# LLNL/ppo_and_friends

Measured on AMD Instinct MI355X. Metric: env_steps_per_sec, higher is better.
Workload: dtype f32; 1 GPU; C2 CartPole-v1 MLP (4->128x3->2 actor, ->1 critic), envs_per_proc=4096, ts_per_rollout=128, fixed-length synthetic trajectories, batch_size=256, epochs_per_iter=10; parallelism=dp1, hip_graphs=True

## Files before the change

### ppo_and_friends_amd/csrc/ppo_update.hip

```cpp
#include "ppo_update_rowpair.hpp"
#include <hip/hip_ext.h>
#include "peer_exchange_device.hpp"
#include <cstdlib>

namespace ppoaf {


template <int HTA, int HTC, bool SPLIT>
__global__ __launch_bounds__(kThreadsU) void ppo_update_fwd_bwd_kernel(UpdateDev u) {
    const int b = blockIdx.x;
    int which = (b >> 2) & 1;
    int g = ((b >> 3) << 2) | (b & 3);
    if (u.confine) {
        const int x = b & 7;
        if ((x >> 2) != u.confine - 1) return;
        which = (x & 3) >> 1;
        g = ((b >> 3) << 1) | (x & 1);
    }
    if (g >= u.n_wg) return;
    if (which == 0) ppo_update_fwd_bwd_body<HTA, SPLIT>(u, 0, g);
    else ppo_update_fwd_bwd_body<HTC, SPLIT>(u, 1, g);
}

template <int HTA, int HTC>
__global__ __launch_bounds__(kThreadsU) void ppo_update_fwd_bwd_pair_kernel(UpdateDev u, PairDev pd) {
    const int b = blockIdx.x, x = b & 7, j = b >> 3;
    int which, g, hf = 0;
    if (u.confine) {
        if ((x >> 2) != u.confine - 1) return;
        which = (x & 3) >> 1;
        if (which == 0 ? HTA == 16 : HTC == 16) { hf = j & 1; g = ((j >> 1) << 1) | (x & 1); }
        else g = (j << 1) | (x & 1);
    } else {
        which = x >> 2;
        if (which == 0 ? HTA == 16 : HTC == 16) { hf = j & 1; g = ((j >> 1) << 2) | (x & 3); }
        else g = (j << 2) | (x & 3);
    }
    if (g >= u.n_wg) return;
    if (which == 0) {
        if constexpr (HTA == 16) ppo_update_fwd_bwd_pair_body<16>(u, 0, g, hf, pd);
        else ppo_update_fwd_bwd_body<HTA, true>(u, 0, g);
    } else {
        if constexpr (HTC == 16) ppo_update_fwd_bwd_pair_body<16>(u, 1, g, hf, pd);
        else ppo_update_fwd_bwd_body<HTC, true>(u, 1, g);
    }
}

constexpr int kRedThreads = 256;

__device__ __forceinline__ void ppo_update_bookkeeping(const UpdateDev& u);

__global__ __launch_bounds__(kRedThreads) void ppo_update_reduce_kernel(UpdateDev u, int compute_norms) {
    __shared__ double red[17];
    if (blockIdx.x == gridDim.x - 1) { ppo_update_bookkeeping(u); return; }
    const long n4 = u.bucket_total >> 2;
    const long idx = (long)blockIdx.x * kRedThreads + threadIdx.x;
    const float4* sl = reinterpret_cast<const float4*>(u.slabs);
    float4 acc = make_float4(0.f, 0.f, 0.f, 0.f);
    if (idx < n4) {
        for (int g0 = 0; g0 < u.n_wg; g0 += 8) {
            float4 v[8];
#pragma unroll
            for (int k = 0; k < 8; ++k)
                v[k] = (g0 + k < u.n_wg) ? sl[(long)(g0 + k) * n4 + idx] : make_float4(0.f, 0.f, 0.f, 0.f);
#pragma unroll
            for (int k = 0; k < 8; ++k) { acc.x += v[k].x; acc.y += v[k].y; acc.z += v[k].z; acc.w += v[k].w; }
        }
// ... 465 lines not shown
```

### ppo_and_friends_amd/csrc/ppo_update_rowtile.hpp

```cpp
#pragma once
#include "ppo_update_dev.hpp"

namespace ppoaf {

extern __shared__ __attribute__((aligned(16))) unsigned char ppo_update_smem[];

#ifdef PPOAF_STAMPS
#ifndef PPOAF_STAMP_BLOCK
#define PPOAF_STAMP_BLOCK 0
#endif
static __device__ unsigned long long g_ppo_update_stamps[2][16];
#define PPOAF_STAMP(k)                                                                   \
    do {                                                                                 \
        if (blockIdx.x == PPOAF_STAMP_BLOCK && threadIdx.x == 0) {                       \
            unsigned long long t_;                                                       \
            asm volatile("s_memtime %0\n\ts_waitcnt lgkmcnt(0)" : "=s"(t_)::"memory");    \
            g_ppo_update_stamps[0][k] = t_;                                              \
        }                                                                                \
    } while (0)
#else
#define PPOAF_STAMP(k) do {} while (0)
#endif



template <int HT, bool NT>
__device__ __forceinline__ void load_fwd_set(const float* __restrict__ W, int n0, int lane, float4 (&fr)[HT]) {
    if constexpr (NT) load_fwd_frags<HT, true>(W, n0, lane, fr);
    else load_fwd_lines_buf<HT>(W, n0, lane, fr);
}
template <int HT, bool NT>
__device__ __forceinline__ f32x4 mfma_fwd_set(const float* __restrict__ A, int HS, int lane, const float4 (&fr)[HT], float init,
                                              float* __restrict__ scratch) {
    if constexpr (NT) return mfma_rows_x_frags<HT>(A, HS, lane, fr, init);
    else return mfma_rows_x_lines<HT>(A, HS, lane, fr, init, scratch);
}

template <int HT, bool SPLIT = false>
__device__ __forceinline__ void ppo_update_fwd_bwd_body(const UpdateDev& u, const int which, const int g) {
    constexpr bool NT = false;
    constexpr long mb_extra = 0;
    constexpr int H = 16 * HT, HS = H + 4;
    int tid_ = threadIdx.x;
    if (NT) {
        asm volatile("" : "+v"(tid_));
        __builtin_assume(tid_ >= 0 && tid_ < kThreadsU);
    }
    const int tid = tid_, lane = tid & 63, wave = NT ? __builtin_amdgcn_readfirstlane(tid >> 6) : (tid >> 6);
    const auto& nd = u.net[which];
    const int in_dim = nd.in_dim, depth = nd.depth, out_dim = nd.out_dim, act = nd.act;
    const int NT0 = (in_dim + 15) >> 4;
    const int INP = 16 * NT0 + 4;
    const float* P = u.params + nd.offset;
    const long B = u.B;
    const long mb = u.cursor[0] + u.mb_offset + mb_extra;
    const long base = mb * u.batch_stride;
    const long szW0 = ((long)H * in_dim + 3) & ~3L;
    auto offW = [&](int l) -> long { return l == 0 ? 0 : szW0 + H + (long)(l - 1) * (H * H + H); };
    auto offB = [&](int l) -> long {
        return l == 0 ? szW0 : offW(l) + (l < depth ? (long)H * H : (((long)out_dim * H + 3) & ~3L));
    };
    float* slab = SPLIT ? u.sp.outpart[which] + (long)g * (nd.size - offW(depth)) - offW(depth)
// ... 7 lines not shown
    };
    const long sp_plane = SPLIT ? (long)u.sp.Bp * H : 0;

    PPOAF_STAMP(0);
    int zl = 0;
    if (NT) asm volatile("" : "+s"(zl));
    float* smem = reinterpret_cast<float*>(ppo_update_smem + zl);
    int* sRow = reinterpret_cast<int*>(smem);
    float* sMisc = smem + 16;
    float* sRowF = smem + 32;
    float* sActF = smem + 80;
    float* sBias = smem + 208;
    float* sWout = sBias + (depth + 1) * H;
    float* sX = sWout + 8 * H;
    float* sH = sX + kRows * INP;
    float* sD0 = sH + (long)depth * kRows * HS;
    float* sD1 = sD0 + kRows * HS;
    float* sOut = sD1 + kRows * HS;
    float* sDOut = sOut + kRows * kMaxOut;
    float* sScr = sDOut + kRows * kMaxOut + wave * 2 * kLineSlot;

    if (!NT && g == 0 && which == 0 && tid == 0) { u.norm_scratch[0] = 0.0; u.norm_scratch[1] = 0.0; }

    const bool has_tile = wave < HT;
    const bool deep = depth == 3 && HT <= kNW;
    float4 fr[HT], fr2[HT];
    const bool l0_pre = in_dim <= 16 && HT <= kNW && has_tile;
    float l0w[4] = {0.f, 0.f, 0.f, 0.f};
    float l2_touch = 0.f;
    constexpr int kCopyRegs = 4;
    float bias_reg[kCopyRegs], wout_reg[kCopyRegs];
    const int n_bias = (depth + 1) * H, n_wout = out_dim * H;
    const bool copy_fits = n_bias <= kCopyRegs * kThreadsU && n_wout <= kCopyRegs * kThreadsU;
    auto request_weights = [&]() {
        if (NT && deep && has_tile) {
            load_fwd_set<HT, NT>(P + offW(1), wave * 16, lane, fr);
            load_fwd_set<HT, NT>(P + offW(2), wave * 16, lane, fr2);
        }
        if (l0_pre) {
            const float* w = P + offW(0) + (long)(wave * 16 + (lane & 15)) * in_dim;
#pragma unroll
            for (int j = 0; j < 4; ++j) { const int k = 4 * j + (lane >> 4); if (k < in_dim) l0w[j] = ld1<NT>(w + k); }
        }
#ifndef PPOAF_L2_TOUCH_MAX_HT
#define PPOAF_L2_TOUCH_MAX_HT 8
#endif
        if (!deep && !NT && HT <= PPOAF_L2_TOUCH_MAX_HT) for (long i = (long)tid * 32; i < nd.size; i += (long)kThreadsU * 32) l2_touch += P[i];
        if (copy_fits) {
#pragma unroll
            for (int r = 0; r < kCopyRegs; ++r) {
                const int i = tid + r * kThreadsU;
                bias_reg[r] = 0.f; wout_reg[r] = 0.f;
                if (i < n_bias) { const int l = i / H, j = i - l * H; if (l < depth || j < out_dim) bias_reg[r] = ld1<NT>(P + offB(l) + j); }
                if (i < n_wout) wout_reg[r] = ld1<NT>(P + offW(depth) + i);
            }
        }
        if (!NT && deep && has_tile) {
            load_fwd_set<HT, NT>(P + offW(1), wave * 16, lane, fr);
            load_fwd_set<HT, NT>(P + offW(2), wave * 16, lane, fr2);
        }
    };
    const float* x_src = which == 0 ? u.obs : u.critic_obs;
    const bool x_pre = !NT && u.pregathered && kRows * in_dim <= 2 * kThreadsU;
    float xr[2] = {0.f, 0.f};
    if (x_pre) {
#pragma unroll
        for (int q = 0; q < 2; ++q) {
            const int idx = tid + q * kThreadsU;
            if (idx < kRows * in_dim && (long)g * kRows + idx / in_dim < B) xr[q] = x_src[(base + (long)g * kRows) * in_dim + idx];
        }
    }
    if (!NT) request_weights();

    if (tid < kRows) {
        const long s = (long)g * kRows + tid;
        int row = -1;
        long di = -1;
        if (s < B) {
            const long p = u.perm[base + s];
            if (p >= 0 && p < u.n_rows) row = u.row_map ? u.row_map[p] : (int)p;
            di = u.pregathered ? base + s : row;
        }
        float av = 0.f, lpo = 0.f, rt = 0.f;
        if (di >= 0) {
            if (which == 0) {
                av = u.adv[di]; lpo = u.old_lp[di];
                if (u.head_kind == PPOAF_HEAD_CATEGORICAL)
                    reinterpret_cast<int*>(sActF)[tid * 8] = (int)reinterpret_cast<const int64_t*>(u.raw_actions)[di];
                else if (u.head_kind == PPOAF_HEAD_MULTI_CATEGORICAL)
                    for (int j = 0; j < u.n_slices; ++j)
                        reinterpret_cast<int*>(sActF)[tid * 8 + j] =
                            (int)reinterpret_cast<const int64_t*>(u.raw_actions)[(long)di * u.n_slices + j];
                else
                    for (int d = 0; d < out_dim; ++d)
                        sActF[tid * 8 + d] = reinterpret_cast<const float*>(u.raw_actions)[(long)di * out_dim + d];
            } else {
                rt = u.rtg[di];
            }
        }
        sRow[tid] = row;
        sRowF[tid] = av; sRowF[16 + tid] = lpo; sRowF[32 + tid] = rt;
    }

    if (tid == 64) {
        if (which == 0) {
            float mean_f = 0.f, std_f = 1.f;
            if (u.normalize_adv) {
                const double* rec = u.adv_records + mb * 3;
                mean_f = (float)rec[1];
                std_f = (float)sqrt(rec[2] / (rec[0] - 1.0));
            }
            sMisc[0] = mean_f; sMisc[1] = std_f;
        } else {
            const int slot = (int)(mb & 1);
            float m = ld1<NT>(u.vn_mean + slot), v = ld1<NT>(u.vn_var + slot);
            double cnt = ld1<NT>(u.vn_count + slot);
            if (u.normalize_values) {
                double n = 0.0, bm = 0.0, M2 = 0.0;
                for (int r = 0; r < u.n_ranks; ++r) {
                    const double* rec = u.vn_records + (mb * u.n_ranks + r) * 3;
                    const double nb = rec[0];
                    if (nb <= 0.0) continue;
                    const double d = rec[1] - bm, nn = n + nb;
                    bm += d * (nb / nn);
                    M2 += rec[2] + d * d * n * nb / nn;
                    n = nn;
                }
                if (n > 0.0) {
                    const float batch_mean = (float)bm, batch_var = (float)(M2 / n);
                    const float delta = batch_mean - m;
                    const double new_count = cnt + n;
                    const float new_mean = (float)((double)m + (double)delta * (n / new_count));
                    const double m_2 = (double)v * cnt + (double)batch_var * n +
                                       (double)(delta * delta) * cnt * n / (cnt + n);
                    m = new_mean; v = (float)(m_2 / (cnt + n)); cnt = new_count;
                }
            }
            sMisc[2] = m; sMisc[3] = v;
            if (g == 0) { u.vn_mean[slot ^ 1] = m; u.vn_var[slot ^ 1] = v; u.vn_count[slot ^ 1] = cnt; }
        }
    }
    if (copy_fits) {
#pragma unroll
        for (int r = 0; r < kCopyRegs; ++r) {
            const int i = tid + r * kThreadsU;
            if (i < n_bias) sBias[i] = bias_reg[r];
            if (i < n_wout) sWout[i] = wout_reg[r];
        }
    } else {
        for (int l = 0; l <= depth; ++l) {
            const int n = (l == depth) ? out_dim : H;
            const float* bb = P + offB(l);
            for (int i = tid; i < n; i += kThreadsU) sBias[l * H + i] = ld1<NT>(bb + i);
        }
        for (int i = tid; i < out_dim * H; i += kThreadsU) sWout[i] = ld1<NT>(P + offW(depth) + i);
    }
    for (int i = tid; i < kRows * INP; i += kThreadsU) sX[i] = 0.f;
    __syncthreads();
    PPOAF_STAMP(1);

    if (x_pre) {
#pragma unroll
        for (int q = 0; q < 2; ++q) {
            const int idx = tid + q * kThreadsU;
            const int s = idx / in_dim, i = idx - s * in_dim;
            if (idx < kRows * in_dim && sRow[s] >= 0) sX[s * INP + i] = xr[q];
        }
    } else {
        const float* src = x_src;
        for (int idx = tid; idx < kRows * in_dim; idx += kThreadsU) {
            const int s = idx / in_dim, i = idx - s * in_dim;
            const int row = sRow[s];
            const long di = u.pregathered ? base + (long)g * kRows + s : row;
            if (row >= 0) sX[s * INP + i] = src[di * in_dim + i];
        }
    }
    if (!deep && depth > 1 && has_tile) load_fwd_set<HT, NT>(P + offW(1), wave * 16, lane, fr);
    __syncthreads();
    PPOAF_STAMP(2);
    if (SPLIT) {
        float* xb = u.sp.xbuf[which] + (long)g * kRows * 64;
        for (int i = tid; i < kRows * 64; i += kThreadsU) {
            const int r = i >> 6, c = i & 63;
            xb[i] = c < 16 * NT0 ? sX[r * INP + c] : 0.f;
        }
    }

    for (int nt = wave; nt < HT; nt += kNW) {
        const int o = nt * 16 + (lane & 15);
        const float bv = sBias[o];
        f32x4 acc = {bv, bv, bv, bv};
        const float* w = P + offW(0) + (long)o * in_dim;
        const float* arow = sX + (lane & 15) * INP;
        for (int k0 = 0; k0 < in_dim; k0 += 16) {
            float bq[4];
#pragma unroll
// ... 159 lines not shown
        if (l == depth - 1) PPOAF_STAMP(12);
        __syncthreads();
        if (l == depth - 1) PPOAF_STAMP(13);
        float* t = Dc; Dc = Dn; Dn = t;
    }
    PPOAF_STAMP(8);

    if (SPLIT) {
        publish_rows(Dc, u.sp.dbuf[which]);
    } else {
        for (int mt = wave; mt < HT; mt += kNW)
            wgrad_mtile(Dc, HS, sX, INP, mt * 16, NT0, in_dim, lane, slab + offW(0), in_dim);
        for (int o = tid; o < H; o += kThreadsU) {
            float acc = 0.f;
#pragma unroll
            for (int s = 0; s < kRows; ++s) acc += Dc[s * HS + o];
            slab[offB(0) + o] = acc;
        }
    }
    if (l2_touch == 1.2345e38f) u.loss_partials[0] = l2_touch;
    PPOAF_STAMP(9);
}

constexpr size_t kRowtileLineFloats = (size_t)kNW * 2 * kLineSlot;
inline size_t rowtile_lds_floats(const NetDev& n) {
    const size_t HS = n.H + 4, INP = 16 * ((n.in_dim + 15) / 16) + 4;
    return 208 + (size_t)(n.depth + 1) * n.H + 8 * (size_t)n.H + kRows * INP + (size_t)n.depth * kRows * HS + 2 * kRows * HS +
           2 * kRows * kMaxOut;
}

}
```

### ppo_and_friends_amd/csrc/ppo_update_tail.hip

```cpp
#include "ppo_update_dev.hpp"
#include "tail_sync.hpp"
#include "peer_exchange_device.hpp"
#include <hip/hip_ext.h>
#include <cstddef>

namespace ppoaf {

constexpr int kTailMaxE = 9;

struct TailBc { long long t; double bc1, bc2s; };
__device__ __forceinline__ TailBc tail_bc_load(const UpdateDev& u, const TailDev& td, const int which) {
    TailBc r;
    r.t = td.ctl->bc_t[which];
    r.bc1 = td.ctl->bc[2 * which];
    r.bc2s = td.ctl->bc[2 * which + 1];
    return r;
}

__device__ __forceinline__ void tail_sync_wave0(const UpdateDev& u, const TailDev& td, const unsigned tag, const int b, const int which,
                                                const long long t_next, const TailBc& pre, const float lr, const double q,
                                                float* s_coef) {
    if (threadIdx.x == 0) tail_publish(td, tag, b, q);
    double bc1 = pre.bc1, bc2s = pre.bc2s;
    if (pre.t != t_next) {
        bc1 = 1.0 - pow((double)u.beta1, (double)t_next);
        bc2s = sqrt(1.0 - pow((double)u.beta2, (double)t_next));
    }
    double sq0, sq1;
    tail_gather(td, tag, sq0, sq1);
    if (threadIdx.x == 0) {
        const float total_norm = (float)sqrt(which ? sq1 : sq0);
        float coef = 1.0f;
        if (u.max_norm > 0.f) coef = fminf(u.max_norm / (total_norm + 1e-6f), 1.0f);
        s_coef[0] = u.grad_scale * coef;
        s_coef[1] = (float)((double)lr / bc1);
        s_coef[2] = (float)bc2s;
    }
}

constexpr int kTailTileFloats = 528;
struct TailXchg { XchgDev x; long long seq, wait_ticks; long seg_base[2]; };

__device__ __forceinline__ __amdgpu_buffer_rsrc_t tail_slot_rsrc(const void* base) {
    return __builtin_amdgcn_make_buffer_rsrc(const_cast<void*>(base), 0, 0xFFFFFFFF, 0x00020000);
}
__device__ __forceinline__ void tail_xchg_publish_wait(const TailXchg& c, const unsigned g) {
    asm volatile("s_waitcnt vmcnt(0)" ::: "memory");
    __syncthreads();
    const XchgDev& x = c.x;
    if (threadIdx.x == 0) {
#pragma unroll
        for (int p = 0; p < kMaxPeers; ++p)
            if (p < x.n_ranks && p != x.rank)
                __hip_atomic_store(&x.peer_flags[p][g * kMaxPeers + x.rank], c.seq, __ATOMIC_RELAXED, __HIP_MEMORY_SCOPE_SYSTEM);
    }
    const int p = (int)threadIdx.x - 64;
    if (p >= 0 && p < x.n_ranks && p != x.rank) {
        long long budget = c.wait_ticks;
        if (__hip_atomic_load(&x.words[3], __ATOMIC_RELAXED, __HIP_MEMORY_SCOPE_AGENT) != 0) budget = 0;
        const long long* flag = &x.my_flags[g * kMaxPeers + p];
        const long long t0 = (long long)wall_clock64();
        while (__hip_atomic_load(flag, __ATOMIC_RELAXED, __HIP_MEMORY_SCOPE_SYSTEM) < c.seq) {
            __builtin_amdgcn_s_sleep(1);
            if ((long long)wall_clock64() - t0 > budget) {
                __hip_atomic_store(&x.words[3], c.seq, __ATOMIC_RELAXED, __HIP_MEMORY_SCOPE_AGENT);
// ... 32 lines not shown
}
__device__ __forceinline__ float tail_xchg_sum1(const TailXchg& c, const long off, const float own) {
    const long fo = (c.seq & 1) * c.x.n4 * 4 + off;
    float acc = 0.f;
#pragma unroll
    for (int p0 = 0; p0 < kMaxPeers; p0 += 8) {
        if (p0 >= c.x.n_ranks) break;
        float v[8];
#pragma unroll
        for (int k = 0; k < 8; ++k) {
            const int p = p0 + k;
            if (p >= c.x.n_ranks) v[k] = 0.f;
            else if (p == c.x.rank) v[k] = own;
            else v[k] = __uint_as_float(__hip_atomic_load(reinterpret_cast<const unsigned*>(reinterpret_cast<const float*>(c.x.peer_slots[p]) + fo),
                                                          __ATOMIC_RELAXED, __HIP_MEMORY_SCOPE_SYSTEM));
        }
#pragma unroll
        for (int k = 0; k < 8; ++k) if (p0 + k < c.x.n_ranks) acc += v[k];
    }
    return acc;
}

struct TailPmv { float p, m, v; };
__device__ __forceinline__ TailPmv tail_pmv_load(const UpdateDev& u, const long idx, const bool ok) {
    TailPmv r = {0.f, 0.f, 0.f};
    if (ok) { r.p = u.params[idx]; r.m = u.exp_avg[idx]; r.v = u.exp_avg_sq[idx]; }
    return r;
}
__device__ __forceinline__ void tail_adam1(const UpdateDev& u, const long idx, const float g, const TailPmv& s, const TailCoef& c) {
    const float gi = g * c.gs;
    const float m = u.beta1 * s.m + (1.0f - u.beta1) * gi;
    const float v = u.beta2 * s.v + (1.0f - u.beta2) * gi * gi;
    const_cast<float*>(u.params)[idx] = s.p - c.step_size * (m / (sqrtf(v) / c.bc2_sqrt + u.adam_eps));
    u.exp_avg[idx] = m;
    u.exp_avg_sq[idx] = v;
}

template <int H, bool XCHG>
__device__ __forceinline__ void tail_job(const UpdateDev& u, const TailDev& td, const unsigned tag, const int b, const int which,
                                         const int job, float* sFold , float* sTile ,
                                         double* s_red, float* s_coef, const TailXchg* xc) {
    constexpr int MAXC = 8;
    const int tid = threadIdx.x, lane = tid & 63;
    const int wave = __builtin_amdgcn_readfirstlane(tid >> 6);
    const auto& nd = u.net[which];
    const int in_dim = nd.in_dim, depth = nd.depth, out_dim = nd.out_dim;
    const int B = (int)u.B;
    const long plane = (long)u.sp.Bp * H;
    const long szW0 = ((long)H * in_dim + 3) & ~3L;
    auto offW = [&](int l) -> long { return l == 0 ? 0 : szW0 + H + (long)(l - 1) * ((long)H * H + H); };
    auto offB = [&](int l) -> long {
        return l == 0 ? szW0 : offW(l) + (l < depth ? (long)H * H : (((long)out_dim * H + 3) & ~3L));
    };
    const long nb = nd.offset;
    float* G = u.grads + nb;
    const long long t_next = (long long)u.step_counts[which] + 1;
    const float lr = u.lr[0];
    const TailBc pre = tail_bc_load(u, td, which);
    constexpr int t = H / 16, t2 = (t + 1) / 2;
    const int n_it0 = (in_dim + 15) / 16, p0 = (n_it0 + 1) / 2;
    const int n_hidden = (depth - 1) * t * t2, n_l0 = t * p0;
    const float sc = u.grad_scale;
    double q = 0.0;
    TAIL_STAMP(td, 0);
    if (job < n_hidden + n_l0) {
        int l, ot, itile, n_it;
        if (job < n_hidden) { l = 1 + job / (t * t2); const int jj = job % (t * t2); ot = jj / t2; itile = 2 * (jj % t2); n_it = t; }
        else { l = 0; const int jj = job - n_hidden; ot = jj / p0; itile = 2 * (jj % p0); n_it = n_it0; }
        const bool two = itile + 1 < n_it;
        const long ldw = l >= 1 ? H : in_dim;
        long eidx[2];
        bool eok[2];
        TailPmv se[2], sb;
#pragma unroll
        for (int k = 0; k < 2; ++k) {
            const int e = tid + 256 * k, row = e >> 5, col = e & 31;
            const int i = itile * 16 + col;
            eok[k] = (col < 16 || two) && i < ldw;
            eidx[k] = nb + offW(l) + (long)(ot * 16 + row) * ldw + i;
            se[k] = tail_pmv_load(u, eidx[k], eok[k]);
        }
        const bool has_b = itile == 0 && tid >= 64 && tid < 80;
        const long bidx = nb + offB(l) + ot * 16 + (tid - 64);
        sb = tail_pmv_load(u, bidx, has_b);
        const long ldx = l >= 1 ? H : 64;
        const __amdgpu_buffer_rsrc_t rd = __builtin_amdgcn_make_buffer_rsrc(u.sp.dbuf[which] + (long)l * plane, 0, 0xFFFFFFFF, 0x00020000);
        const __amdgpu_buffer_rsrc_t rx = __builtin_amdgcn_make_buffer_rsrc(
            l >= 1 ? u.sp.hbuf[which] + (long)(l - 1) * plane : u.sp.xbuf[which], 0, 0xFFFFFFFF, 0x00020000);
        const unsigned dl = 4u * (unsigned)((lane >> 4) * H + ot * 16 + (lane & 15));
        const unsigned xl = 4u * (unsigned)((lane >> 4) * (int)ldx + itile * 16 + (lane & 15));
        const int nc = (B + 15) >> 4;
        float a[MAXC][4], x0[MAXC][4], x1[MAXC][4];
#pragma unroll
        for (int c = 0; c < MAXC; ++c) {
            const int ch = wave + 4 * c;
#pragma unroll
            for (int j = 0; j < 4; ++j) { a[c][j] = 0.f; x0[c][j] = 0.f; x1[c][j] = 0.f; }
            if (ch < nc) {
#pragma unroll
                for (int j = 0; j < 4; ++j) {
                    const unsigned sd = 4u * (unsigned)((16 * ch + 4 * j) * H), sx = 4u * (unsigned)((16 * ch + 4 * j) * (int)ldx);
                    a[c][j] = __uint_as_float(__builtin_amdgcn_raw_buffer_load_b32(rd, dl, sd, 0));
                    x0[c][j] = __uint_as_float(__builtin_amdgcn_raw_buffer_load_b32(rx, xl, sx, 0));
                    if (two) x1[c][j] = __uint_as_float(__builtin_amdgcn_raw_buffer_load_b32(rx, xl + 64u, sx, 0));
                }
            }
        }
        TAIL_STAMP(td, 1);
        tail_f32x4 acc0 = {0.f, 0.f, 0.f, 0.f}, acc1 = {0.f, 0.f, 0.f, 0.f};
        float bsum = 0.f;
#pragma unroll
        for (int c = 0; c < MAXC; ++c) {
            if (wave + 4 * c < nc) {
#pragma unroll
                for (int j = 0; j < 4; ++j) {
                    acc0 = __builtin_amdgcn_mfma_f32_16x16x4f32(a[c][j], x0[c][j], acc0, 0, 0, 0);
                    if (two) acc1 = __builtin_amdgcn_mfma_f32_16x16x4f32(a[c][j], x1[c][j], acc1, 0, 0, 0);
                    bsum += a[c][j];
                }
            }
        }
        TAIL_STAMP(td, 2);
        if (wave > 0) {
            *reinterpret_cast<tail_f32x4*>(sFold + (((wave - 1) * 2 + 0) * 64 + lane) * 4) = acc0;
            *reinterpret_cast<tail_f32x4*>(sFold + (((wave - 1) * 2 + 1) * 64 + lane) * 4) = acc1;
        }
        bsum += __shfl_xor(bsum, 16, 64);
        bsum += __shfl_xor(bsum, 32, 64);
        if (lane < 16) sFold[1536 + wave * 16 + lane] = bsum;
        __syncthreads();
// ... 17 lines not shown
        }
        if (XCHG) {
            __syncthreads();
            const bool mine = tid < 128 || (itile == 0 && tid < 132);
            const long off = (long)b * kTailTileFloats + 4 * tid;
            tail_f32x4 own = {0.f, 0.f, 0.f, 0.f};
            if (mine) {
                own = *reinterpret_cast<const tail_f32x4*>(sTile + 4 * tid);
                tail_xchg_store4(*xc, off, own);
            }
            tail_xchg_publish_wait(*xc, (unsigned)b);
            if (mine) *reinterpret_cast<tail_f32x4*>(sTile + 4 * tid) = tail_xchg_sum4(*xc, off, own);
            __syncthreads();
            if (wave == 0) {
#pragma unroll
                for (int r = 0; r < 4; ++r) {
                    const int row = 4 * (lane >> 4) + r;
                    acc0[r] = sTile[row * 32 + (lane & 15)];
                    acc1[r] = sTile[row * 32 + 16 + (lane & 15)];
                }
                if (lane < 16) bg = sTile[512 + lane];
            }
        }
        if (wave == 0) {
#pragma unroll
            for (int r = 0; r < 4; ++r) {
                if (i < ldw) q += (double)(acc0[r] * sc) * (acc0[r] * sc);
                if (two && i + 16 < ldw) q += (double)(acc1[r] * sc) * (acc1[r] * sc);
            }
            if (itile == 0 && lane < 16) q += (double)(bg * sc) * (bg * sc);
            TAIL_STAMP(td, 3);
            q = tail_wave_sum(q);
            TAIL_STAMP(td, 4);
            tail_sync_wave0(u, td, tag, b, which, t_next, pre, lr, q, s_coef);
        }
        __syncthreads();
        TAIL_STAMP(td, 5);
        const TailCoef cf = {s_coef[0], s_coef[1], s_coef[2]};
#pragma unroll
        for (int k = 0; k < 2; ++k)
            if (eok[k]) tail_adam1(u, eidx[k], sTile[tid + 256 * k], se[k], cf);
        if (has_b) tail_adam1(u, bidx, sTile[512 + tid - 64], sb, cf);
#pragma unroll
        for (int k = 0; k < 2; ++k)
            if (eok[k]) u.grads[eidx[k]] = sTile[tid + 256 * k];
        if (has_b) u.grads[bidx] = sTile[512 + tid - 64];
        TAIL_STAMP(td, 6);
    } else {
        const long seg_off = offW(depth), seg_len = nd.size - seg_off;
        const float* outpart = u.sp.outpart[which];
        const int n_hb = (B + 15) >> 4;
        TailPmv se[kTailMaxE];
        float ge[kTailMaxE];
#pragma unroll
        for (int k = 0; k < kTailMaxE; ++k) {
            const long idx = tid + (long)kWgradThreads * k;
            se[k] = tail_pmv_load(u, nb + seg_off + idx, idx < seg_len);
            ge[k] = 0.f;
        }
#pragma unroll
        for (int k = 0; k < kTailMaxE; ++k) {
            const long idx = tid + (long)kWgradThreads * k;
            if (idx < seg_len) {
                float acc = 0.f;
                for (int g0 = 0; g0 < n_hb; g0 += 8) {
                    float pv[8];
#pragma unroll
                    for (int kk = 0; kk < 8; ++kk) pv[kk] = outpart[(long)(g0 + kk < n_hb ? g0 + kk : 0) * seg_len + idx];
#pragma unroll
                    for (int kk = 0; kk < 8; ++kk) if (g0 + kk < n_hb) acc += pv[kk];
                }
                ge[k] = acc;
            }
        }
        if (XCHG) {
#pragma unroll
            for (int k = 0; k < kTailMaxE; ++k) {
                const long idx = tid + (long)kWgradThreads * k;
                if (idx < seg_len) tail_xchg_store1(*xc, xc->seg_base[which] + idx, ge[k]);
            }
            tail_xchg_publish_wait(*xc, (unsigned)b);
#pragma unroll
            for (int k = 0; k < kTailMaxE; ++k) {
                const long idx = tid + (long)kWgradThreads * k;
                if (idx < seg_len) ge[k] = tail_xchg_sum1(*xc, xc->seg_base[which] + idx, ge[k]);
            }
        }
#pragma unroll
        for (int k = 0; k < kTailMaxE; ++k) {
            const long idx = tid + (long)kWgradThreads * k;
            if (idx < seg_len) {
                G[seg_off + idx] = ge[k];
                q += (double)(ge[k] * sc) * (ge[k] * sc);
            }
        }
        q = tail_wave_sum(q);
        if (lane == 0) s_red[wave] = q;
        __syncthreads();
        if (wave == 0) {
            q = tail_wave_sum(lane < 4 ? s_red[lane] : 0.0);
            tail_sync_wave0(u, td, tag, b, which, t_next, pre, lr, q, s_coef);
        }
        __syncthreads();
        const TailCoef cf = {s_coef[0], s_coef[1], s_coef[2]};
#pragma unroll
        for (int k = 0; k < kTailMaxE; ++k) {
            const long idx = tid + (long)kWgradThreads * k;
            if (idx < seg_len) tail_adam1(u, nb + seg_off + idx, ge[k], se[k], cf);
        }
    }
}

template <int HA, int HC, bool XCHG>
__global__ __launch_bounds__(kWgradThreads) void ppo_update_wgrad_adam_kernel(UpdateDev u, TailDev td, TailXchg xc) {
    __shared__ double s_red[17];
    __shared__ __attribute__((aligned(16))) float s_fold[6 * 256 + 64];
    __shared__ float s_tile[16 * 32 + 16];
    __shared__ float s_coef[4];
    const int b = blockIdx.x;
    const unsigned long long seq = __hip_atomic_load(&td.ctl->seq, __ATOMIC_RELAXED, __HIP_MEMORY_SCOPE_AGENT);
    const unsigned tag = ((unsigned)seq & 0x7fffffffu) + 1u;
    if (b == td.nblk) {
        if (threadIdx.x >= 64) return;
        ppo_update_bookkeeping_totals(u);
        const int w = threadIdx.x & 1;
        const long long t_now = (long long)u.step_counts[w] + 1;
        double c_now[2] = {0.0, 0.0}, c_next[2] = {0.0, 0.0};
        if (threadIdx.x < 2) {
            c_now[0] = 1.0 - pow((double)u.beta1, (double)t_now);
            c_now[1] = sqrt(1.0 - pow((double)u.beta2, (double)t_now));
            c_next[0] = 1.0 - pow((double)u.beta1, (double)(t_now + 1));
            c_next[1] = sqrt(1.0 - pow((double)u.beta2, (double)(t_now + 1)));
        }
        double sq0, sq1;
        tail_gather(td, tag, sq0, sq1);
        if (threadIdx.x < 2) {
            u.step_counts[w] = t_now;
            u.norm_scratch[2 + 2 * w] = c_now[0];
            u.norm_scratch[3 + 2 * w] = c_now[1];
            td.ctl->bc_t[w] = t_now + 1;
            td.ctl->bc[2 * w] = c_next[0];
            td.ctl->bc[2 * w + 1] = c_next[1];
        }
        if (threadIdx.x == 0) {
            __hip_atomic_store(&td.ctl->seq, seq + 1ull, __ATOMIC_RELAXED, __HIP_MEMORY_SCOPE_AGENT);
            if (u.cursor_advance) u.cursor[0] += u.cursor_advance;
        }
        return;
    }
    const int job = (b & 7) * td.per_xcd + (b >> 3);
    const bool live = job < td.jobs_a + td.jobs_c;
    if (XCHG && live) xc.seq = xchg_sequence(xc.x, (unsigned)b);
    if (job < td.jobs_a) tail_job<HA, XCHG>(u, td, tag, b, 0, job, s_fold, s_tile, s_red, s_coef, &xc);
    else if (live) tail_job<HC, XCHG>(u, td, tag, b, 1, job - td.jobs_a, s_fold, s_tile, s_red, s_coef, &xc);
    else if (threadIdx.x == 0) tail_publish(td, tag, b, 0.0);
    if (XCHG && live) xchg_advance(xc.x, xc.seq, (unsigned)b);
}

template <int HA, int HC, bool XCHG>
static int tail_launch_as(const UpdateDev& u, const TailDev& td, const TailXchg& xc, hipStream_t s, hipEvent_t e0, hipEvent_t e1) {
    const int rc = require_all_resident(reinterpret_cast<const void*>(ppo_update_wgrad_adam_kernel<HA, HC, XCHG>), kWgradThreads,
                                        td.nblk + 1, "ppo_update_wgrad_adam");
    if (rc) return rc;
    if (e0 || e1)
        hipExtLaunchKernelGGL((ppo_update_wgrad_adam_kernel<HA, HC, XCHG>), dim3((unsigned)(td.nblk + 1)), dim3(kWgradThreads), 0, s, e0, e1, 0, u, td, xc);
    else
        hipLaunchKernelGGL((ppo_update_wgrad_adam_kernel<HA, HC, XCHG>), dim3((unsigned)(td.nblk + 1)), dim3(kWgradThreads), 0, s, u, td, xc);
    return check_launch("ppo_update_wgrad_adam");
}
template <int HA, int HC>
static int tail_launch(const UpdateDev& u, const TailDev& td, const TailXchg* xc, hipStream_t s, hipEvent_t e0, hipEvent_t e1) {
    if (xc) return tail_launch_as<HA, HC, true>(u, td, *xc, s, e0, e1);
    return tail_launch_as<HA, HC, false>(u, td, TailXchg(), s, e0, e1);
}

static int tail_dispatch(const UpdateDev& u, const TailDev& td, const TailXchg* xc, hipStream_t s, hipEvent_t e0, hipEvent_t e1) {
    const int ha = u.net[0].H, hc = u.net[1].H;
    if (ha == 32 && hc == 32) return tail_launch<32, 32>(u, td, xc, s, e0, e1);
    if (ha == 64 && hc == 64) return tail_launch<64, 64>(u, td, xc, s, e0, e1);
    if (ha == 128 && hc == 128) return tail_launch<128, 128>(u, td, xc, s, e0, e1);
    if (ha == 256 && hc == 256) return tail_launch<256, 256>(u, td, xc, s, e0, e1);
    if (ha == 128 && hc == 256) return tail_launch<128, 256>(u, td, xc, s, e0, e1);
    if (ha == 64 && hc == 128) return tail_launch<64, 128>(u, td, xc, s, e0, e1);
    set_error("ppo_update_wgrad_adam: hidden widths (actor %d, critic %d) not instantiated", ha, hc);
    return PPOAF_E_INVALID;
}

static int tail_prepare(const ppoaf_ppo_update_args_t* args, void* ctl, double wait_seconds, UpdateDev& u, TailDev& td) {
    int rc = make_update_dev(args, u);
    if (rc) return rc;
    PPOAF_REQUIRE(u.split, "ppo_update_wgrad_adam: args->split_workspace is not set (the tail of the split-wgrad chain)");
    PPOAF_REQUIRE(ctl && (((uintptr_t)ctl) & 63) == 0, "ppo_update_wgrad_adam: control block missing or not 64-byte aligned");
    PPOAF_REQUIRE(wait_seconds > 0.0 && wait_seconds <= 600.0, "ppo_update_wgrad_adam: wait_seconds=%g", wait_seconds);
    td.ctl = reinterpret_cast<TailCtl*>(ctl);
    td.budget = (long long)(wait_seconds * 1.0e8);
    td.jobs_a = split_wgrad_jobs(u.net[0]);
    td.jobs_c = split_wgrad_jobs(u.net[1]);
    td.per_xcd = split_wgrad_per_xcd(u);
    td.nblk = split_wgrad_blocks(u);
    PPOAF_REQUIRE(td.nblk <= 64 * kTailMaxRounds, "ppo_update_wgrad_adam: %d workgroups, a polling wave holds %d records", td.nblk,
                  64 * kTailMaxRounds);
    for (int w = 0; w < 2; ++w)
        PPOAF_REQUIRE(ws_seg_len(u.net[w]) <= (long)kWgradThreads * kTailMaxE, "ppo_update_wgrad_adam: output segment of %ld floats (at most %d)",
                      ws_seg_len(u.net[w]), kWgradThreads * kTailMaxE);
    return PPOAF_OK;
}

static long tail_exchange_floats(const UpdateDev& u, long* seg_base) {
    long off = (long)split_wgrad_blocks(u) * kTailTileFloats;
    for (int w = 0; w < 2; ++w) {
        if (seg_base) seg_base[w] = off;
        off += (ws_seg_len(u.net[w]) + 3) & ~3L;
    }
    return off;
}

// ... 62 lines not shown
```

Baseline: 1.085 million env-steps/s.

## Hoist row scalars, stats and Adam control loads ahead of compute in update kernels

The forward/backward body now issues per-row scalar loads (advantages, old log-probs, actions, returns), normalisation records and hidden-layer weight sets earlier, with a specialised 'tables' path for depth-3 pregathered inputs without a row map. Kernel arguments are pinned into scalar registers up front. The wgrad+Adam tail uses buffer loads for params and moments and defers the sequence, step and bias-correction loads until after the gradient loads are in flight. The aim is to hide memory latency on these small kernels, at the cost of more register pressure and a new 32-bit offset limit on the bucket size.

```diff
diff --git a/ppo_and_friends_amd/csrc/ppo_update.hip b/ppo_and_friends_amd/csrc/ppo_update.hip
--- a/ppo_and_friends_amd/csrc/ppo_update.hip
+++ b/ppo_and_friends_amd/csrc/ppo_update.hip
@@ -8,7 +8,7 @@
 
 template <int HTA, int HTC, bool SPLIT>
 __global__ __launch_bounds__(kThreadsU) void ppo_update_fwd_bwd_kernel(UpdateDev u) {
-    const int b = blockIdx.x;
+    const int b = rowtile_request_args(u, blockIdx.x);
     int which = (b >> 2) & 1;
     int g = ((b >> 3) << 2) | (b & 3);
     if (u.confine) {
@@ -39,10 +39,10 @@
     if (g >= u.n_wg) return;
     if (which == 0) {
         if constexpr (HTA == 16) ppo_update_fwd_bwd_pair_body<16>(u, 0, g, hf, pd);
-        else ppo_update_fwd_bwd_body<HTA, true>(u, 0, g);
+        else ppo_update_fwd_bwd_body_as<HTA, true, false>(u, 0, g);
     } else {
         if constexpr (HTC == 16) ppo_update_fwd_bwd_pair_body<16>(u, 1, g, hf, pd);
-        else ppo_update_fwd_bwd_body<HTC, true>(u, 1, g);
+        else ppo_update_fwd_bwd_body_as<HTC, true, false>(u, 1, g);
     }
 }
 
diff --git a/ppo_and_friends_amd/csrc/ppo_update_rowtile.hpp b/ppo_and_friends_amd/csrc/ppo_update_rowtile.hpp
--- a/ppo_and_friends_amd/csrc/ppo_update_rowtile.hpp
+++ b/ppo_and_friends_amd/csrc/ppo_update_rowtile.hpp
@@ -36,8 +36,30 @@
     else return mfma_rows_x_lines<HT>(A, HS, lane, fr, init, scratch);
 }
 
-template <int HT, bool SPLIT = false>
-__device__ __forceinline__ void ppo_update_fwd_bwd_body(const UpdateDev& u, const int which, const int g) {
+__device__ __forceinline__ int rowtile_request_args(const UpdateDev& u, int b) {
+    const NetDev& a = u.net[0];
+    const NetDev& c = u.net[1];
+    asm("" : "+s"(b)
+        : "s"(a.in_dim), "s"(a.H), "s"(a.depth), "s"(a.out_dim), "s"(a.act), "s"((&a.act)[1]), "s"(a.offset), "s"(a.size), "s"(a.log_std_off),
+          "s"(c.in_dim), "s"(c.H), "s"(c.depth), "s"(c.out_dim), "s"(c.act), "s"((&c.act)[1]), "s"(c.offset), "s"(c.size), "s"(c.log_std_off),
+          "s"(u.params), "s"(u.norm_scratch), "s"(u.head_kind),
+          "s"(u.obs), "s"(u.critic_obs), "s"(u.raw_actions), "s"(u.adv), "s"(u.old_lp), "s"(u.rtg), "s"(u.values), "s"(u.perm),
+          "s"(u.row_map), "s"(u.n_rows), "s"(u.cursor), "s"(u.B), "s"(u.batch_stride), "s"(u.mb_offset), "s"(u.cursor_advance),
+          "s"(u.normalize_values), "s"(u.n_ranks), "s"(u.vn_mean), "s"(u.vn_var), "s"(u.vn_count), "s"(u.vn_records),
+          "s"(u.adv_records), "s"(u.normalize_adv), "s"(u.use_huber), "s"(u.pregathered), "s"(u.surr_clip),
+          "s"(u.n_wg), "s"(u.confine));
+    const long cur = u.cursor[0];
+    asm("" : "+s"(b)
+        : "s"(cur), "s"(u.entropy_weight), "s"(u.kl_loss_weight), "s"(u.huber_delta), "s"(u.min_std), "s"(u.loss_partials),
+          "s"(u.sp.hbuf[0]), "s"(u.sp.hbuf[1]), "s"(u.sp.dbuf[0]), "s"(u.sp.dbuf[1]), "s"(u.sp.outpart[0]), "s"(u.sp.outpart[1]),
+          "s"(u.sp.xbuf[0]), "s"(u.sp.xbuf[1]), "s"(u.sp.W), "s"(u.sp.xcc[0]), "s"(u.sp.xcc[1]), "s"(u.sp.Bp), "s"(u.n_slices),
+          "s"(u.slices[0]), "s"(u.slices[1]), "s"(u.slices[2]), "s"(u.slices[3]), "s"(u.slices[4]), "s"(u.slices[5]),
+          "s"(u.slices[6]), "s"(u.slices[7]));
+    return b;
+}
+
+template <int HT, bool SPLIT, bool TABLES>
+__device__ __forceinline__ void ppo_update_fwd_bwd_body_as(const UpdateDev& u, const int which, const int g) {
     constexpr bool NT = false;
     constexpr long mb_extra = 0;
     constexpr int H = 16 * HT, HS = H + 4;
@@ -91,8 +113,9 @@
 
     if (!NT && g == 0 && which == 0 && tid == 0) { u.norm_scratch[0] = 0.0; u.norm_scratch[1] = 0.0; }
 
-    const bool has_tile = wave < HT;
-    const bool deep = depth == 3 && HT <= kNW;
+    const bool has_tile = HT >= kNW || wave < HT;
+    static_assert(!TABLES || HT <= kNW, "deep prefetch: one output tile per wave");
+    const bool deep = TABLES || (depth == 3 && HT <= kNW);
     float4 fr[HT], fr2[HT];
     const bool l0_pre = in_dim <= 16 && HT <= kNW && has_tile;
     float l0w[4] = {0.f, 0.f, 0.f, 0.f};
@@ -124,13 +147,15 @@
                 if (i < n_wout) wout_reg[r] = ld1<NT>(P + offW(depth) + i);
             }
         }
+    };
+    auto request_hidden_sets = [&]() {
         if (!NT && deep && has_tile) {
             load_fwd_set<HT, NT>(P + offW(1), wave * 16, lane, fr);
             load_fwd_set<HT, NT>(P + offW(2), wave * 16, lane, fr2);
         }
     };
     const float* x_src = which == 0 ? u.obs : u.critic_obs;
-    const bool x_pre = !NT && u.pregathered && kRows * in_dim <= 2 * kThreadsU;
+    const bool x_pre = !NT && (TABLES || u.pregathered) && kRows * in_dim <= 2 * kThreadsU;
     float xr[2] = {0.f, 0.f};
     if (x_pre) {
 #pragma unroll
@@ -139,62 +164,135 @@
             if (idx < kRows * in_dim && (long)g * kRows + idx / in_dim < B) xr[q] = x_src[(base + (long)g * kRows) * in_dim + idx];
         }
     }
+    if constexpr (TABLES) asm volatile("; ppoaf_rowtile_tables_prologue");
     if (!NT) request_weights();
 
+    constexpr int kActRegs = 8;
+    constexpr int kVnPre = 2;
+    const bool row_lane = tid < kRows && (long)g * kRows + tid < B;
+    static_assert(!TABLES || !NT, "per-epoch tables: separate launches only");
+    constexpr bool early = TABLES;
+    const int n_act = which != 0 ? 0 : u.head_kind == PPOAF_HEAD_CATEGORICAL ? 1
+                    : u.head_kind == PPOAF_HEAD_MULTI_CATEGORICAL ? u.n_slices : out_dim;
+    long perm_v = -1;
+    float av = 0.f, lpo = 0.f, rt = 0.f;
+    int act_bits[kActRegs];
+#pragma unroll
+    for (int j = 0; j < kActRegs; ++j) act_bits[j] = 0;
+    auto request_row_scalars = [&](const long di) {
+        if (which == 0) {
+            av = u.adv[di]; lpo = u.old_lp[di];
+            if (u.head_kind == PPOAF_HEAD_CATEGORICAL) {
+                act_bits[0] = (int)reinterpret_cast<const int64_t*>(u.raw_actions)[di];
+            } else if (u.head_kind == PPOAF_HEAD_MULTI_CATEGORICAL) {
+#pragma unroll
+                for (int j = 0; j < kActRegs; ++j)
+                    if (j < n_act) act_bits[j] = (int)reinterpret_cast<const int64_t*>(u.raw_actions)[(long)di * u.n_slices + j];
+            } else {
+#pragma unroll
+                for (int d = 0; d < kActRegs; ++d)
+                    if (d < n_act) act_bits[d] = __float_as_int(reinterpret_cast<const float*>(u.raw_actions)[(long)di * out_dim + d]);
+            }
+        } else {
+            rt = u.rtg[di];
+        }
+    };
+    if (row_lane) {
+        const long s = (long)g * kRows + tid;
+        perm_v = u.perm[base + s];
+        if (early) request_row_scalars(base + s);
+    }
+    const bool stat_lane = tid == 64;
+    double adv_rec[3] = {0.0, 0.0, 0.0}, vn_rec[kVnPre][3];
+    float vn_m = 0.f, vn_v = 0.f;
+    double vn_cnt = 0.0;
+#pragma unroll
+    for (int r = 0; r < kVnPre; ++r) { vn_rec[r][0] = 0.0; vn_rec[r][1] = 0.0; vn_rec[r][2] = 0.0; }
+    if (stat_lane) {
+        if (which == 0) {
+            if (u.normalize_adv) {
+                const double* rec = u.adv_records + mb * 3;
+                adv_rec[0] = rec[0]; adv_rec[1] = rec[1]; adv_rec[2] = rec[2];
+            }
+        } else {
+            const int slot = (int)(mb & 1);
+            vn_m = ld1<NT>(u.vn_mean + slot); vn_v = ld1<NT>(u.vn_var + slot);
+            vn_cnt = ld1<NT>(u.vn_count + slot);
+            if (u.normalize_values) {
+#pragma unroll
+                for (int r = 0; r < kVnPre; ++r) {
+                    if (r < u.n_ranks) {
+                        const double* rec = u.vn_records + (mb * u.n_ranks + r) * 3;
+                        vn_rec[r][0] = rec[0]; vn_rec[r][1] = rec[1]; vn_rec[r][2] = rec[2];
+                    }
+                }
+            }
+        }
+    }
+    double vn_n = 0.0, vn_bm = 0.0, vn_M2 = 0.0;
+    auto vn_merge = [&](const double nb, const double mean, const double m2) {
+        if (nb <= 0.0) return;
+        const double d = mean - vn_bm, nn = vn_n + nb;
+        vn_bm += d * (nb / nn);
+        vn_M2 += m2 + d * d * vn_n * nb / nn;
+        vn_n = nn;
+    };
+    if (stat_lane && which != 0 && u.normalize_values && u.n_ranks > kVnPre) {
+#pragma unroll
+        for (int r = 0; r < kVnPre; ++r) vn_merge(vn_rec[r][0], vn_rec[r][1], vn_rec[r][2]);
+        for (int r = kVnPre; r < u.n_ranks; ++r) {
+            const double* rec = u.vn_records + (mb * u.n_ranks + r) * 3;
+            vn_merge(rec[0], rec[1], rec[2]);
+        }
+    }
+    if (!NT) request_hidden_sets();
+
     if (tid < kRows) {
-        const long s = (long)g * kRows + tid;
-        int row = -1;
-        long di = -1;
-        if (s < B) {
-            const long p = u.perm[base + s];
-            if (p >= 0 && p < u.n_rows) row = u.row_map ? u.row_map[p] : (int)p;
-            di = u.pregathered ? base + s : row;
-        }
-        float av = 0.f, lpo = 0.f, rt = 0.f;
-        if (di >= 0) {
-            if (which == 0) {
-                av = u.adv[di]; lpo = u.old_lp[di];
-                if (u.head_kind == PPOAF_HEAD_CATEGORICAL)
-                    reinterpret_cast<int*>(sActF)[tid * 8] = (int)reinterpret_cast<const int64_t*>(u.raw_actions)[di];
-                else if (u.head_kind == PPOAF_HEAD_MULTI_CATEGORICAL)
-                    for (int j = 0; j < u.n_slices; ++j)
-                        reinterpret_cast<int*>(sActF)[tid * 8 + j] =
-                            (int)reinterpret_cast<const int64_t*>(u.raw_actions)[(long)di * u.n_slices + j];
-                else
-                    for (int d = 0; d < out_dim; ++d)
-                        sActF[tid * 8 + d] = reinterpret_cast<const float*>(u.raw_actions)[(long)di * out_dim + d];
-            } else {
-                rt = u.rtg[di];
-            }
-        }
-        sRow[tid] = row;
-        sRowF[tid] = av; sRowF[16 + tid] = lpo; sRowF[32 + tid] = rt;
-    }
-
-    if (tid == 64) {
+        auto store_row = [&](const int row, const bool have) {
+            if (have) {
+#pragma unroll
+                for (int j = 0; j < kActRegs; ++j)
+                    if (j < n_act) reinterpret_cast<int*>(sActF)[tid * 8 + j] = act_bits[j];
+            }
+            sRow[tid] = row;
+            sRowF[tid] = av; sRowF[16 + tid] = lpo; sRowF[32 + tid] = rt;
+        };
+        if constexpr (TABLES) {
+            int row = -1;
+            if (row_lane && perm_v >= 0 && perm_v < u.n_rows) row = (int)perm_v;
+            store_row(row, row_lane);
+        } else {
+            int row = -1;
+            long di = -1;
+            if (row_lane) {
+                const long p = perm_v;
+                if (p >= 0 && p < u.n_rows) row = u.row_map ? u.row_map[p] : (int)p;
+                di = u.pregathered ? base + (long)g * kRows + tid : row;
+            }
+            if (di >= 0 && !early) request_row_scalars(di);
+            store_row(row, di >= 0);
+        }
+    }
+
+    if (stat_lane) {
         if (which == 0) {
             float mean_f = 0.f, std_f = 1.f;
             if (u.normalize_adv) {
-                const double* rec = u.adv_records + mb * 3;
-                mean_f = (float)rec[1];
-                std_f = (float)sqrt(rec[2] / (rec[0] - 1.0));
+                mean_f = (float)adv_rec[1];
+                std_f = (float)sqrt(adv_rec[2] / (adv_rec[0] - 1.0));
             }
             sMisc[0] = mean_f; sMisc[1] = std_f;
         } else {
             const int slot = (int)(mb & 1);
-            float m = ld1<NT>(u.vn_mean + slot), v = ld1<NT>(u.vn_var + slot);
-            double cnt = ld1<NT>(u.vn_count + slot);
+            float m = vn_m, v = vn_v;
+            double cnt = vn_cnt;
             if (u.normalize_values) {
-                double n = 0.0, bm = 0.0, M2 = 0.0;
-                for (int r = 0; r < u.n_ranks; ++r) {
-                    const double* rec = u.vn_records + (mb * u.n_ranks + r) * 3;
-                    const double nb = rec[0];
-                    if (nb <= 0.0) continue;
-                    const double d = rec[1] - bm, nn = n + nb;
-                    bm += d * (nb / nn);
-                    M2 += rec[2] + d * d * n * nb / nn;
-                    n = nn;
+                if (u.n_ranks <= kVnPre) {
+#pragma unroll
+                    for (int r = 0; r < kVnPre; ++r)
+                        if (r < u.n_ranks) vn_merge(vn_rec[r][0], vn_rec[r][1], vn_rec[r][2]);
                 }
+                const double n = vn_n, bm = vn_bm, M2 = vn_M2;
                 if (n > 0.0) {
                     const float batch_mean = (float)bm, batch_var = (float)(M2 / n);
                     const float delta = batch_mean - m;
@@ -240,7 +338,7 @@
         for (int idx = tid; idx < kRows * in_dim; idx += kThreadsU) {
             const int s = idx / in_dim, i = idx - s * in_dim;
             const int row = sRow[s];
-            const long di = u.pregathered ? base + (long)g * kRows + s : row;
+            const long di = (TABLES || u.pregathered) ? base + (long)g * kRows + s : row;
             if (row >= 0) sX[s * INP + i] = src[di * in_dim + i];
         }
     }
@@ -446,6 +544,17 @@
     PPOAF_STAMP(9);
 }
 
+template <int HT, bool SPLIT = false>
+__device__ __forceinline__ void ppo_update_fwd_bwd_body(const UpdateDev& u, const int which, const int g) {
+    if constexpr (HT <= kNW) {
+        if (u.net[which].depth == 3 && u.pregathered && !u.row_map) {
+            ppo_update_fwd_bwd_body_as<HT, SPLIT, true>(u, which, g);
+            return;
+        }
+    }
+    ppo_update_fwd_bwd_body_as<HT, SPLIT, false>(u, which, g);
+}
+
 constexpr size_t kRowtileLineFloats = (size_t)kNW * 2 * kLineSlot;
 inline size_t rowtile_lds_floats(const NetDev& n) {
     const size_t HS = n.H + 4, INP = 16 * ((n.in_dim + 15) / 16) + 4;
diff --git a/ppo_and_friends_amd/csrc/ppo_update_tail.hip b/ppo_and_friends_amd/csrc/ppo_update_tail.hip
--- a/ppo_and_friends_amd/csrc/ppo_update_tail.hip
+++ b/ppo_and_friends_amd/csrc/ppo_update_tail.hip
@@ -9,20 +9,45 @@
 constexpr int kTailMaxE = 9;
 
 struct TailBc { long long t; double bc1, bc2s; };
-__device__ __forceinline__ TailBc tail_bc_load(const UpdateDev& u, const TailDev& td, const int which) {
-    TailBc r;
-    r.t = td.ctl->bc_t[which];
-    r.bc1 = td.ctl->bc[2 * which];
-    r.bc2s = td.ctl->bc[2 * which + 1];
+
+constexpr bool kTailOneTrip(const int ha, const int hc) { return ha <= 128 && hc <= 128; }
+struct TailPre { unsigned long long seq; long long t; float lr; TailBc bc; };
+__device__ __forceinline__ TailPre tail_pre_load(const UpdateDev& u, const TailDev& td, const int which, const unsigned long long seq) {
+    TailPre r;
+    r.seq = seq;
+    r.t = (long long)u.step_counts[which];
+    r.lr = u.lr[0];
+    r.bc.t = td.ctl->bc_t[which];
+    r.bc.bc1 = td.ctl->bc[2 * which];
+    r.bc.bc2s = td.ctl->bc[2 * which + 1];
     return r;
 }
-
-__device__ __forceinline__ void tail_sync_wave0(const UpdateDev& u, const TailDev& td, const unsigned tag, const int b, const int which,
-                                                const long long t_next, const TailBc& pre, const float lr, const double q,
-                                                float* s_coef) {
+__device__ __forceinline__ TailPre tail_pre_request(const UpdateDev& u, const TailDev& td, const int which) {
+    TailPre r;
+    r.seq = __hip_atomic_load(&td.ctl->seq, __ATOMIC_RELAXED, __HIP_MEMORY_SCOPE_AGENT);
+    r.t = __hip_atomic_load(&u.step_counts[which], __ATOMIC_RELAXED, __HIP_MEMORY_SCOPE_WORKGROUP);
+    r.lr = __hip_atomic_load(&u.lr[0], __ATOMIC_RELAXED, __HIP_MEMORY_SCOPE_WORKGROUP);
+    r.bc.t = __hip_atomic_load(&td.ctl->bc_t[which], __ATOMIC_RELAXED, __HIP_MEMORY_SCOPE_WORKGROUP);
+    r.bc.bc1 = __hip_atomic_load(&td.ctl->bc[2 * which], __ATOMIC_RELAXED, __HIP_MEMORY_SCOPE_WORKGROUP);
+    r.bc.bc2s = __hip_atomic_load(&td.ctl->bc[2 * which + 1], __ATOMIC_RELAXED, __HIP_MEMORY_SCOPE_WORKGROUP);
+    return r;
+}
+__device__ __forceinline__ TailPre tail_pre_use(TailPre r) {
+    asm volatile("" : "+v"(r.seq), "+v"(r.t), "+v"(r.lr), "+v"(r.bc.t), "+v"(r.bc.bc1), "+v"(r.bc.bc2s));
+    return r;
+}
+__device__ __forceinline__ unsigned tail_tag(const unsigned long long seq) {
+    return ((unsigned)seq & 0x7fffffffu) + 1u;
+}
+
+__device__ __forceinline__ void tail_sync_wave0(const UpdateDev& u, const TailDev& td, const int b, const int which,
+                                                const TailPre& pre , const double q, float* s_coef) {
+    const unsigned tag = tail_tag(pre.seq);
+    const long long t_next = pre.t + 1;
+    const float lr = pre.lr;
     if (threadIdx.x == 0) tail_publish(td, tag, b, q);
-    double bc1 = pre.bc1, bc2s = pre.bc2s;
-    if (pre.t != t_next) {
+    double bc1 = pre.bc.bc1, bc2s = pre.bc.bc2s;
+    if (pre.bc.t != t_next) {
         bc1 = 1.0 - pow((double)u.beta1, (double)t_next);
         bc2s = sqrt(1.0 - pow((double)u.beta2, (double)t_next));
     }
@@ -41,6 +66,11 @@
 constexpr int kTailTileFloats = 528;
 struct TailXchg { XchgDev x; long long seq, wait_ticks; long seg_base[2]; };
 
+__device__ __forceinline__ long long tail_xchg_sequence(const TailXchg& c, const unsigned g) {
+    long long v = c.x.group_seq[g];
+    asm volatile("" : "+v"(v));
+    return v + 1;
+}
 __device__ __forceinline__ __amdgpu_buffer_rsrc_t tail_slot_rsrc(const void* base) {
     return __builtin_amdgcn_make_buffer_rsrc(const_cast<void*>(base), 0, 0xFFFFFFFF, 0x00020000);
 }
@@ -119,9 +149,19 @@
 }
 
 struct TailPmv { float p, m, v; };
+__device__ __forceinline__ unsigned tail_pmv_off(const long idx) { return 4u * (unsigned)idx; }
+__device__ __forceinline__ void tail_pmv_hold(const unsigned off) { asm volatile("" :: "v"(off)); }
+template <bool ONE_TRIP>
 __device__ __forceinline__ TailPmv tail_pmv_load(const UpdateDev& u, const long idx, const bool ok) {
     TailPmv r = {0.f, 0.f, 0.f};
-    if (ok) { r.p = u.params[idx]; r.m = u.exp_avg[idx]; r.v = u.exp_avg_sq[idx]; }
+    if constexpr (!ONE_TRIP) {
+        if (ok) { r.p = u.params[idx]; r.m = u.exp_avg[idx]; r.v = u.exp_avg_sq[idx]; }
+    } else if (ok) {
+        const unsigned off = tail_pmv_off(idx);
+        r.p = __uint_as_float(__builtin_amdgcn_raw_buffer_load_b32(tail_slot_rsrc(u.params), off, 0, 0));
+        r.m = __uint_as_float(__builtin_amdgcn_raw_buffer_load_b32(tail_slot_rsrc(u.exp_avg), off, 0, 0));
+        r.v = __uint_as_float(__builtin_amdgcn_raw_buffer_load_b32(tail_slot_rsrc(u.exp_avg_sq), off, 0, 0));
+    }
     return r;
 }
 __device__ __forceinline__ void tail_adam1(const UpdateDev& u, const long idx, const float g, const TailPmv& s, const TailCoef& c) {
@@ -133,10 +173,10 @@
     u.exp_avg_sq[idx] = v;
 }
 
-template <int H, bool XCHG>
-__device__ __forceinline__ void tail_job(const UpdateDev& u, const TailDev& td, const unsigned tag, const int b, const int which,
+template <int H, bool XCHG, bool ONE_TRIP>
+__device__ __forceinline__ void tail_job(const UpdateDev& u, const TailDev& td, const unsigned long long seq0, const int b, const int which,
                                          const int job, float* sFold , float* sTile ,
-                                         double* s_red, float* s_coef, const TailXchg* xc) {
+                                         double* s_red, float* s_coef, TailXchg* xc) {
     constexpr int MAXC = 8;
     const int tid = threadIdx.x, lane = tid & 63;
     const int wave = __builtin_amdgcn_readfirstlane(tid >> 6);
@@ -151,14 +191,13 @@
     };
     const long nb = nd.offset;
     float* G = u.grads + nb;
-    const long long t_next = (long long)u.step_counts[which] + 1;
-    const float lr = u.lr[0];
-    const TailBc pre = tail_bc_load(u, td, which);
     constexpr int t = H / 16, t2 = (t + 1) / 2;
     const int n_it0 = (in_dim + 15) / 16, p0 = (n_it0 + 1) / 2;
     const int n_hidden = (depth - 1) * t * t2, n_l0 = t * p0;
     const float sc = u.grad_scale;
     double q = 0.0;
+    TailPre pre;
+    if constexpr (!ONE_TRIP) pre = tail_pre_load(u, td, which, seq0);
     TAIL_STAMP(td, 0);
     if (job < n_hidden + n_l0) {
         int l, ot, itile, n_it;
@@ -175,11 +214,11 @@
             const int i = itile * 16 + col;
             eok[k] = (col < 16 || two) && i < ldw;
             eidx[k] = nb + offW(l) + (long)(ot * 16 + row) * ldw + i;
-            se[k] = tail_pmv_load(u, eidx[k], eok[k]);
+            se[k] = tail_pmv_load<ONE_TRIP>(u, eidx[k], eok[k]);
         }
         const bool has_b = itile == 0 && tid >= 64 && tid < 80;
         const long bidx = nb + offB(l) + ot * 16 + (tid - 64);
-        sb = tail_pmv_load(u, bidx, has_b);
+        sb = tail_pmv_load<ONE_TRIP>(u, bidx, has_b);
         const long ldx = l >= 1 ? H : 64;
         const __amdgpu_buffer_rsrc_t rd = __builtin_amdgcn_make_buffer_rsrc(u.sp.dbuf[which] + (long)l * plane, 0, 0xFFFFFFFF, 0x00020000);
         const __amdgpu_buffer_rsrc_t rx = __builtin_amdgcn_make_buffer_rsrc(
@@ -203,6 +242,13 @@
                 }
             }
         }
+#pragma unroll
+        for (int k = 0; k < 2; ++k) if constexpr (ONE_TRIP) tail_pmv_hold(tail_pmv_off(eidx[k]));
+        if constexpr (ONE_TRIP) tail_pmv_hold(tail_pmv_off(bidx));
+        if constexpr (ONE_TRIP) {
+            pre = tail_pre_request(u, td, which);
+            if (XCHG) xc->seq = tail_xchg_sequence(*xc, (unsigned)b);
+        }
         TAIL_STAMP(td, 1);
         tail_f32x4 acc0 = {0.f, 0.f, 0.f, 0.f}, acc1 = {0.f, 0.f, 0.f, 0.f};
         float bsum = 0.f;
@@ -266,6 +312,7 @@
                 if (lane < 16) bg = sTile[512 + lane];
             }
         }
+        const TailPre got = ONE_TRIP ? tail_pre_use(pre) : pre;
         if (wave == 0) {
 #pragma unroll
             for (int r = 0; r < 4; ++r) {
@@ -276,7 +323,7 @@
             TAIL_STAMP(td, 3);
             q = tail_wave_sum(q);
             TAIL_STAMP(td, 4);
-            tail_sync_wave0(u, td, tag, b, which, t_next, pre, lr, q, s_coef);
+            tail_sync_wave0(u, td, b, which, got, q, s_coef);
         }
         __syncthreads();
         TAIL_STAMP(td, 5);
@@ -299,8 +346,12 @@
 #pragma unroll
         for (int k = 0; k < kTailMaxE; ++k) {
             const long idx = tid + (long)kWgradThreads * k;
-            se[k] = tail_pmv_load(u, nb + seg_off + idx, idx < seg_len);
+            se[k] = tail_pmv_load<ONE_TRIP>(u, nb + seg_off + idx, idx < seg_len);
             ge[k] = 0.f;
+        }
+        if constexpr (ONE_TRIP) {
+            pre = tail_pre_request(u, td, which);
+            if (XCHG) xc->seq = tail_xchg_sequence(*xc, (unsigned)b);
         }
 #pragma unroll
         for (int k = 0; k < kTailMaxE; ++k) {
@@ -341,9 +392,10 @@
         q = tail_wave_sum(q);
         if (lane == 0) s_red[wave] = q;
         __syncthreads();
+        const TailPre got = ONE_TRIP ? tail_pre_use(pre) : pre;
         if (wave == 0) {
             q = tail_wave_sum(lane < 4 ? s_red[lane] : 0.0);
-            tail_sync_wave0(u, td, tag, b, which, t_next, pre, lr, q, s_coef);
+            tail_sync_wave0(u, td, b, which, got, q, s_coef);
         }
         __syncthreads();
         const TailCoef cf = {s_coef[0], s_coef[1], s_coef[2]};
@@ -361,11 +413,14 @@
     __shared__ __attribute__((aligned(16))) float s_fold[6 * 256 + 64];
     __shared__ float s_tile[16 * 32 + 16];
     __shared__ float s_coef[4];
+    constexpr bool ONE_TRIP = kTailOneTrip(HA, HC);
     const int b = blockIdx.x;
-    const unsigned long long seq = __hip_atomic_load(&td.ctl->seq, __ATOMIC_RELAXED, __HIP_MEMORY_SCOPE_AGENT);
-    const unsigned tag = ((unsigned)seq & 0x7fffffffu) + 1u;
+    unsigned long long seq0 = 0;
+    if constexpr (!ONE_TRIP) seq0 = __hip_atomic_load(&td.ctl->seq, __ATOMIC_RELAXED, __HIP_MEMORY_SCOPE_AGENT);
     if (b == td.nblk) {
         if (threadIdx.x >= 64) return;
+        const unsigned long long seq = ONE_TRIP ? __hip_atomic_load(&td.ctl->seq, __ATOMIC_RELAXED, __HIP_MEMORY_SCOPE_AGENT) : seq0;
+        const unsigned tag = tail_tag(seq);
         ppo_update_bookkeeping_totals(u);
         const int w = threadIdx.x & 1;
         const long long t_now = (long long)u.step_counts[w] + 1;
@@ -394,10 +449,11 @@
     }
     const int job = (b & 7) * td.per_xcd + (b >> 3);
     const bool live = job < td.jobs_a + td.jobs_c;
-    if (XCHG && live) xc.seq = xchg_sequence(xc.x, (unsigned)b);
-    if (job < td.jobs_a) tail_job<HA, XCHG>(u, td, tag, b, 0, job, s_fold, s_tile, s_red, s_coef, &xc);
-    else if (live) tail_job<HC, XCHG>(u, td, tag, b, 1, job - td.jobs_a, s_fold, s_tile, s_red, s_coef, &xc);
-    else if (threadIdx.x == 0) tail_publish(td, tag, b, 0.0);
+    if (XCHG && !ONE_TRIP && live) xc.seq = xchg_sequence(xc.x, (unsigned)b);
+    if (job < td.jobs_a) tail_job<HA, XCHG, ONE_TRIP>(u, td, seq0, b, 0, job, s_fold, s_tile, s_red, s_coef, &xc);
+    else if (live) tail_job<HC, XCHG, ONE_TRIP>(u, td, seq0, b, 1, job - td.jobs_a, s_fold, s_tile, s_red, s_coef, &xc);
+    else if (threadIdx.x == 0)
+        tail_publish(td, tail_tag(ONE_TRIP ? __hip_atomic_load(&td.ctl->seq, __ATOMIC_RELAXED, __HIP_MEMORY_SCOPE_AGENT) : seq0), b, 0.0);
     if (XCHG && live) xchg_advance(xc.x, xc.seq, (unsigned)b);
 }
 
@@ -436,6 +492,8 @@
     PPOAF_REQUIRE(u.split, "ppo_update_wgrad_adam: args->split_workspace is not set (the tail of the split-wgrad chain)");
     PPOAF_REQUIRE(ctl && (((uintptr_t)ctl) & 63) == 0, "ppo_update_wgrad_adam: control block missing or not 64-byte aligned");
     PPOAF_REQUIRE(wait_seconds > 0.0 && wait_seconds <= 600.0, "ppo_update_wgrad_adam: wait_seconds=%g", wait_seconds);
+    PPOAF_REQUIRE(u.bucket_total < (1L << 30), "ppo_update_wgrad_adam: bucket of %ld floats (32-bit byte offsets: fewer than 2^30)",
+                  (long)u.bucket_total);
     td.ctl = reinterpret_cast<TailCtl*>(ctl);
     td.budget = (long long)(wait_seconds * 1.0e8);
     td.jobs_a = split_wgrad_jobs(u.net[0]);
```

Result: faster. 1.128 million env-steps/s, median of 6 (+4.0%).
